# ianwhale/tblup

Hardware: AMD Instinct MI355X
Metric: GBLUP fitness evals/sec (whole node), 2k×50k SNP, DE pop=256; 1/2/4/8 GPUs (higher is better)
Workload: dtype fp4 e2m1 system tiles (exact integer genotype products, fp32 accumulate) + f64 Cholesky/solve; 1 GPU; config2: 2000 animals x 50000 SNPs, panel k=1000, DE pop 256 (256 per GPU), n_train=1280, n_valid=320, h2=0.4; pop_total=256, pop_per_gpu=256, parallelism=population sharded over 1 GPU(s) (strong scaling)

## Files before the change

tblup_amd/csrc/capi.hip:

```cpp
#include <algorithm>
#include <cmath>
#include <cstdio>
#include <cstdlib>
#include <cstring>
#include <map>
#include <memory>
#include <string>
#include <unordered_map>
#include <vector>

#include "capi_ctx.h"
#include "mt_jump.h"

using namespace tblup;

namespace tblup_capi {

thread_local std::string g_err;

int fail(int code, const std::string& msg) {
  g_err = msg;
  return code;
}

// ... 423 lines not shown
  const double tri = (double)d.nT * (d.nT + 1) / 2.0 + (double)d.nV * d.nT;
  for (int64_t b = 0; b < B; ++b) {
    const int64_t k = h_off[b + 1] - h_off[b];
    grm_flops += 2.0 * (double)k * tri;
    gather_bytes += 0.5 * (double)k * (double)(d.nT + d.nV);
    stats_bytes += 16.0 * (double)k;
  }
  const int64_t pk_row = (sd.form == FORM_DUAL) ? dual_pk_row(sd) : 0;
  const int64_t pstride = sd.prow * pk_row;
  uint8_t* panel = cv.take<uint8_t>((size_t)B * pstride);
  double* u = cv.take<double>((size_t)B * sd.prow);
  double* scal = cv.take<double>((size_t)B * SCAL);
  double* L = cv.take<double>((size_t)B * l_stride(sd.NT));
  double* Dinv = cv.take<double>((size_t)B * sd.NT * NPACK * BLKD);
  double* z = cv.take<double>((size_t)B * d.nt * sd.ns);
  double* wv = cv.take<double>((size_t)B * d.nt * sd.ns);
  double* rhs = cv.take<double>((size_t)B * d.nt * sd.ns);
  double* Sp = cv.take<double>((size_t)B * TBLUP_NSLOT * 36 * 256);
  const bool use_st = sys_tiles(c, d, sd) && rq.mode != ChunkMode::DebugK && !ft.gsh;
  double* Kdg = cv.take<double>((size_t)B * sd.NT * NPACK * BLKD);
  int16_t* kdb = use_st ? cv.take<int16_t>((size_t)B * sd.NT * KD_TILE) : nullptr;
  int16_t* kcb = use_st ? cv.take<int16_t>((size_t)B * sd.NT * (sd.NT - 1) / 2 * KC_TILE) : nullptr;
  double* Pp = uses_part(c, B, sd.NT, sys_tiles(c, d, sd)) ? cv.take<double>((size_t)2 * B * sd.NT * TILE * TILE) : nullptr;
  double* Qb = use_last_term(c, sd, B) ? cv.take<double>((size_t)B * NPACK * BLKD) : nullptr;
  const bool fold_share = use_st && sd.form == FORM_PRIMAL && ft.nf > 1 && ft.share;
  if (int rc = ws_check(c, cv)) return rc;
  cl.d = d; cl.sd = sd; cl.B = B; cl.off = rq.d_off; cl.idx = rq.d_idx;
  cl.L = L; cl.Dinv = Dinv; cl.z = z; cl.w = wv; cl.rhs = rhs; cl.S = Sp; cl.u = u; cl.scal = scal;
  cl.Kd = Kdg; cl.kd = kdb; cl.kc = kcb; cl.part = Pp; cl.q = Qb;
  cl.yT = (const double*)rq.sp->yT.p; cl.panel = panel; cl.pstride = pstride; cl.gs_row = d.nRp; cl.gpk_row = d.nRp / 4;
  cl.skip = dbg_skip(c) | (rq.mode == ChunkMode::DebugL ? FLAG_WRITE_LJJ : 0);
  cl.padskip = (sd.form == FORM_PRIMAL && sd.pad_first) ? 1 : 0;
  cl.sys_st = c->sys_st;
  std::vector<OffPlan> plan(sd.NT);
  for (int J = 0; J < sd.NT; ++J) {
    plan[J] = plan_of(c, B, sd.NT, J, use_st);
    if (ft.gsh) plan[J].ne = 0;
  }
  const int32_t* csA = (const int32_t*)c->colsum_all.p;
  const bool fuse_stats = !redo && use_st && sd.form == FORM_PRIMAL && (fold_share || sys_tiles_grid(cl) > 0);
  const StatsFuse sf{csA, d.n, d.nT, rq.branch, rq.h2, rq.d_h2, (int32_t*)c->status.p + ST_INDEX, scal, u, rhs};
  int rc = 0;
  if (!redo && !fuse_stats)
    rc = timed(c, s, KC_STATS, 2.0 * (double)h_off[B], stats_bytes, [&] {
      return launch_indiv_stats(d_idx, d_off, B, ft, csA, d, sd, rq.branch, rq.h2, rq.d_h2, scal, u, rhs,
                                (int32_t*)c->status.p + ST_INDEX, s);
    });
  if (rc) return rc;
  if (sd.form == FORM_DUAL && !redo) {
    rc = timed(c, s, KC_GATHER, 0.0, gather_bytes, [&] {
      return launch_gather(ft, d_idx, d_off, pstride, B, csA, scal, d, pk_row, panel, u, s);
    });
    if (rc) return rc;
  }
  res.z = z;
  if (rq.mode == ChunkMode::DebugK) {
    double* K = cv.take<double>((size_t)B * d.nRp * d.nTp);
    if (int rc2 = ws_check(c, cv)) return rc2;
    res.K = K;
    const double kbytes = (double)B * ((double)d.nT * d.nT / 2.0 + (double)d.nV * d.nT) * 8.0;
    return timed(c, s, KC_GRM, grm_flops, kbytes + gather_bytes / 2.0,
                 [&] { return launch_grm(panel, pstride, pk_row, d_off, u, scal, d, B, K, s); });
  }
  res.K = L;
  const double T3 = (double)TILE * TILE * TILE;
  uint64_t* wgt = nullptr;
// ... 180 lines not shown
  if (hipGetDeviceCount(&ndev) != hipSuccess || ndev == 0) return fail(TBLUP_ERR_HIP, "no HIP device available");
  if (device < 0 || device >= ndev) return fail(TBLUP_ERR_ARG, "device id out of range");
  HIPCHK(hipSetDevice(device));
  std::unique_ptr<tblup_ctx> c(new tblup_ctx());
  c->device = device;
  c->n = n;
  c->P = P;
  if (panel) c->pheno.assign(pheno, pheno + n);
  c->nt = 1;
  HIPCHK(hipStreamCreateWithFlags(&c->stream, hipStreamNonBlocking));
  const char* env = getenv("TBLUP_WORKSPACE_MB");
  c->budget = (size_t)(env ? atoll(env) : 32768) << 20;
#ifdef TBLUP_DIAG_BUILD
  const char* dbg = getenv("TBLUP_DBG_SKIP");
  c->dbg_skip = dbg ? atoi(dbg) : 0;
#endif
  const char* wt = getenv("TBLUP_WG_TRACE");
  c->wg_trace = wt && atoi(wt) != 0;
  const char* fp = getenv("TBLUP_FORM");
  c->form_pref = fp ? std::max(0, std::min(2, atoi(fp))) : 0;
  if (const char* e = getenv("TBLUP_AHEAD")) c->ahead = std::max(-1, std::min(1, atoi(e)));
  if (const char* e = getenv("TBLUP_SOLVE_CHAIN")) c->solve_chain = std::max(-1, std::min(1, atoi(e)));
  if (const char* e = getenv("TBLUP_SOLVE_PULL")) c->solve_pull = std::max(-1, std::min(1, atoi(e)));
  if (const char* e = getenv("TBLUP_CHAIN_SYNC")) c->chain_sync = atoi(e);
  if (const char* e = getenv("TBLUP_LAST_TERM")) c->last_term = std::max(-1, std::min(1, atoi(e)));
  if (const char* e = getenv("TBLUP_LT_MASK")) c->lt_mask = (int)strtol(e, nullptr, 0);
  if (const char* e = getenv("TBLUP_FOLD_FUSE")) c->fold_fuse = atoi(e) != 0;
  if (const char* e = getenv("TBLUP_FOLD_SHARE")) c->fold_share = atoi(e) != 0;
  if (const char* e = getenv("TBLUP_SYS_ST")) c->sys_st = std::max(-1, std::min(1, atoi(e)));
  if (const char* e = getenv("TBLUP_FOLD_GSHARE")) c->fold_gshare = atoi(e) != 0;
  if (const char* e = getenv("TBLUP_DUAL_ST")) c->dual_st = atoi(e) != 0;
  if (const char* e = getenv("TBLUP_DIAG_D")) c->diag_d = std::max(-1, std::min(1, atoi(e)));
  if (const char* e = getenv("TBLUP_DIAG_E")) c->diag_e = std::max(-1, std::min(2, atoi(e)));
  if (const char* e = getenv("TBLUP_PAD_FIRST")) c->pad_first = atoi(e) != 0;
  if (const char* e = getenv("TBLUP_RELIAB_LDS")) c->reliab_lds = atoi(e) != 0;
  if (const char* e = getenv("TBLUP_SCORE_LDS")) c->score_lds = atoi(e) != 0;
  if (const char* e = getenv("TBLUP_NRS")) c->nrs = (atoi(e) == 1 || atoi(e) == 2 || atoi(e) == 4) ? atoi(e) : 0;
  if (const char* e = getenv("TBLUP_CHAIN_DEBUG")) {
    int sp = 0, dl = 0, sh = 0;
    if (sscanf(e, "%d,%d,%d", &sp, &dl, &sh) == 3 && sp > 0 && dl >= 0 && sh > 0) {
      c->chain_dbg_spin = sp;
      c->chain_dbg_delay = dl;
      c->chain_dbg_shots = sh;
    }
  }
  if (!panel) {
    *out = c.release();
    return 0;
  }
  const size_t gbytes = (size_t)n * (size_t)P;
  if (int rc = dev_alloc(c.get(), c->geno_sm, gbytes)) return rc;
  if (int rc = dev_alloc(c.get(), c->colsum_all, (size_t)P * 4)) return rc;
  if (int rc = dev_alloc(c.get(), c->status, ST_WORDS * 4)) return rc;
  HIPCHK(hipMemsetAsync(c->status.p, 0, ST_WORDS * 4, c->stream));
  if (layout == TBLUP_LAYOUT_SNP_MAJOR) {
    HIPCHK(hipMemcpyAsync(c->geno_sm.p, geno, gbytes, hipMemcpyHostToDevice, c->stream));
  } else {
    if (int rc = dev_alloc(c.get(), c->scratch, gbytes)) return rc;
    HIPCHK(hipMemcpyAsync(c->scratch.p, geno, gbytes, hipMemcpyHostToDevice, c->stream));
    HIPCHK(launch_transpose_geno((const int8_t*)c->scratch.p, (int8_t*)c->geno_sm.p, n, P, c->stream));
  }
  HIPCHK(launch_colsum_all((const int8_t*)c->geno_sm.p, (int32_t*)c->colsum_all.p, n, P, c->stream));
  HIPCHK(hipStreamSynchronize(c->stream));
  dev_free(c.get(), c->scratch);
  *out = c.release();
  return 0;
// ... 639 lines not shown
```

tblup_amd/csrc/capi_ctx.h:

```cpp
#pragma once
#include <functional>
#include <map>
#include <memory>
#include <string>
#include <vector>

#include "../../include/tblup_gpu.h"
#include "tblup_internal.h"

struct tblup_ctx;

namespace tblup_capi {

int fail(int code, const std::string& msg);

#define HIPCHK(expr)                                                                                      \
  do {                                                                                                    \
    hipError_t e_ = (expr);                                                                               \
    if (e_ != hipSuccess) return fail(TBLUP_ERR_HIP, std::string(#expr) + ": " + hipGetErrorString(e_)); \
  } while (0)

inline int64_t round_up(int64_t x, int64_t m) { return (x + m - 1) / m * m; }

struct DevBuf {
// ... 41 lines not shown
  DevBuf dec_keys, dec_idx;
  DevBuf de_polys, de_small, de_par, de_chi;
  int64_t de_L = -1, de_pop = -1;
  bool de_end_jump = false;
  uint32_t* de_host = nullptr;
  char* de_stage = nullptr;
  size_t de_stage_bytes = 0;
  hipEvent_t de_ev = nullptr;
  bool de_pending = false;
  DevBuf mde_dev;
  std::vector<uint32_t> mde_key;
  int32_t mde_pos = -1;
  int64_t mde_cmax = 0;
  int64_t mde_pop = -1, mde_L = -1, mde_scr = 0;
  size_t budget = 0;
  bool profiling = false;
  std::vector<EventPair> pending;
  std::vector<hipEvent_t> event_pool;
  double ms[TBLUP_N_KCLASS] = {0};
  int64_t launches[TBLUP_N_KCLASS] = {0};
  double flops[TBLUP_N_KCLASS] = {0};
  double bytes[TBLUP_N_KCLASS] = {0};
  int64_t mem_in_use = 0;

  bool wg_trace = false;
  DevBuf wgt;
  int64_t wgt_used = 0;
  int dbg_skip = 0;
  int form_pref = 0;
  int ahead = -1;
  int nrs = 0;
  int diag_d = -1;
  int diag_e = -1;
  int chain_sync = 0;
  int last_term = -1;
  int lt_mask = -1;
  int solve_chain = -1;
  int solve_pull = -1;
  int fold_fuse = 1;
  int fold_share = 1;
  int fold_gshare = 1;
  int dual_st = 1;
  std::vector<int32_t> gmap_host;
  int sys_st = -1;
  int pad_first = 1;
  int reliab_lds = 1;
  int score_lds = 1;
  std::vector<int64_t> fold_hoff;
  DevBuf chain;
  int32_t chain_seq = 0;
  bool host_entry = false;
  int64_t chain_recoveries = 0;
  int32_t chain_dbg_spin = 0, chain_dbg_delay = 0, chain_dbg_shots = 0;
};

namespace tblup_capi {
int dev_alloc(tblup_ctx* c, DevBuf& b, size_t bytes);
void dev_free(tblup_ctx* c, DevBuf& b);
int check_ctx(tblup_ctx* c);
void clear_error();

struct Carve {
  char* base;
  size_t used = 0;
  template <typename T>
  T* take(size_t count) {
// ... 48 lines not shown
```

tblup_amd/csrc/k_chol.hip:

```cpp
#include "chol_dev.h"
#include <algorithm>
#include <type_traits>

namespace tblup {

namespace {

constexpr int BKD = 16;
constexpr int LTS = BKD * TILE;
constexpr int TT = TILE * TILE;

__device__ __forceinline__ v4d mfma64(double a, double b, v4d c) {
  return __builtin_amdgcn_mfma_f64_16x16x4f64(a, b, c, 0, 0, 0);
}
__device__ __forceinline__ v4d mfma64_nega(double a, double b, v4d c) {
  return __builtin_amdgcn_mfma_f64_16x16x4f64(a, b, c, 0, 0, 1);
}

constexpr int NSLOT = TBLUP_NSLOT;

typedef __attribute__((address_space(3))) void* lds_ptr_t;


__device__ __forceinline__ int lt_off(int k, int x) { return k * TILE + 2 * ((x >> 1) ^ (8 * (k & 1))) + (x & 1); }
// ... 138 lines not shown
                                         double* dst) {
  const int l = threadIdx.x & 63;
  const double* sc = a.scal + b * SCAL;
  const double sa = sc[SC_SA], cN = sc[SC_CN], invd = sc[SC_INVD], lam = sc[SC_LAM], sm = sc[SC_SM];
  const int64_t nrow = (int64_t)sc[SC_NROW], pad = (int64_t)sc[SC_PAD];
  int q, sb;
  tri_decode(e, q, sb);
  const int64_t j0 = (int64_t)J * TILE;
  const double* ub = a.u + b * a.prow + j0;
  const int il = 16 * sb + (l & 15);
  const int64_t gj = j0 + il;
  const double uj = ub[il];
  const v4i c4 = unpack_counts4(cv);
#pragma unroll
  for (int r = 0; r < 4; ++r) {
    const int cl = 16 * q + (l >> 4) + 4 * r;
    const int64_t gi = j0 + cl;
    const double kv = grm_value(c4[r], ub[cl], uj, sa, cN, invd, sm);
    const double v = (sys_real(gi, pad, nrow) && sys_real(gj, pad, nrow)) ? kv + ((gi == gj) ? lam : 0.0)
                                                                         : ((gi == gj) ? 1.0 : 0.0);
    double* d = dst + pk(q, sb) + bo((l >> 4) + 4 * r, l & 15);
    __builtin_nontemporal_store(v - sub[r], d);
  }
}
__device__ __forceinline__ int2 kd_load(const CholArgs& a, int64_t b, int J, int e) {
  const int l = threadIdx.x & 63;
  return nt_load2(a.kd + kd_tile(a.NT, b, J) + (e * 64 + l) * 4);
}

__device__ __forceinline__ int skip_rows(const CholArgs& a, int64_t b) {
  return a.padskip ? ((int)a.scal[b * SCAL + SC_PAD] & ~3) : 0;
}

__device__ __forceinline__ void factor16_any(const CholArgs& a, double* D, double* X, int l, uint64_t* st = nullptr) {
  if (a.skip & FLAG_WRITE_LJJ)
    factor16<true>(D, X, l, st);
  else
    factor16<false>(D, X, l, st);
}

__device__ __forceinline__ void dstamp(const CholArgs& a, int slot) {
  if (a.dtr && blockIdx.x == 0 && (threadIdx.x & 63) == 0)
    a.dtr[(threadIdx.x >> 6) * 64 + slot] = __builtin_amdgcn_s_memrealtime();
}

__device__ __forceinline__ int32_t gsh_count(const CholArgs& a, int64_t s, int64_t r, int64_t c) {
  const FoldTab& ft = a.ft;
  const int32_t* mp = ft.gmap + (int64_t)fold_of(ft, s) * ft.gmap_ld;
  const int32_t mr = mp[r], mc = mp[c];
  return (mr >= 0 && mc >= 0) ? ft.gsh[((s % ft.bpf) * ft.gsh_ld + mr) * ft.gsh_ld + mc] : 0;
}

constexpr int DW = 8;
constexpr int DTHR = 64 * DW;
static_assert(DTHR == 4 * TILE, "diag z: four lanes per row");

constexpr int OW = 8;
constexpr int OTH = 64 * OW;

template <int D, int WCL = -1>
__device__ __forceinline__ void i8_tt8_pk64(const uint8_t* sa, const uint8_t* sb, int64_t nblk, uint8_t* lds,
                                            v4i (&cnt)[8]) {
  const int l = threadIdx.x & 63, w = threadIdx.x >> 6;
  const int wc = (WCL < 0) ? w : WCL;
#pragma unroll
  for (int cb = 0; cb < 8; ++cb) cnt[cb] = v4i{0, 0, 0, 0};
  if (nblk <= 0) return;
  const int64_t nst = (nblk + 3) >> 2;
  constexpr int TB = TILE * 64;
  auto issue = [&](int64_t st) {
    uint8_t* slot = lds + (int)(st % D) * 2 * TB;
    glds16_asm(sa + st * 64, slot + w * 1024);
    glds16_asm(sb + st * 64, slot + TB + w * 1024);
  };
  for (int64_t st = 0; st < D - 1 && st < nst; ++st) issue(st);
  const int rho = l & 15, prow = (rho >> 2) + 4 * (rho & 3), ch = l >> 4;
  const int tail_ch = (int)(nblk & 3);
  for (int64_t st = 0; st < nst; ++st) {
    if (st + D - 2 < nst) {
      asm volatile("s_waitcnt vmcnt(%0)" ::"n"((D - 2) * 2) : "memory");
    } else {
      asm volatile("s_waitcnt vmcnt(0)" ::: "memory");
    }
    __builtin_amdgcn_s_barrier();
    if (st + D - 1 < nst) issue(st + D - 1);
    const uint8_t* As = lds + (int)(st % D) * 2 * TB;
    const uint8_t* Bs = As + TB;
    uint4 bq = *reinterpret_cast<const uint4*>(Bs + i8off_b(16 * wc + rho, ch));
// ... 316 lines not shown
  for (; lb + 1 < q; lb += 2) {
    const double* A0 = Tp + pk(q, lb);
    const double* B0 = Xp + pk(lb, jb);
    const double* A1 = Tp + pk(q, lb + 1);
    const double* B1 = Xp + pk(lb + 1, jb);
#pragma unroll
    for (int kk = 0; kk < 4; ++kk) {
      const int k = 4 * kk + (l >> 4);
      s0 = mfma64(A0[bo(l & 15, k)], B0[bo(k, l & 15)], s0);
      s1 = mfma64(A1[bo(l & 15, k)], B1[bo(k, l & 15)], s1);
    }
  }
  if (lb < q) {
    const double* A0 = Tp + pk(q, lb);
    const double* B0 = Xp + pk(lb, jb);
#pragma unroll
    for (int kk = 0; kk < 4; ++kk) {
      const int k = 4 * kk + (l >> 4);
      s0 = mfma64(A0[bo(l & 15, k)], B0[bo(k, l & 15)], s0);
    }
  }
  const v4d sacc = s0 + s1;
  v4d xo = {0.0, 0.0, 0.0, 0.0};
  const double* Xqq = Xp + pk(q, q);
#pragma unroll
  for (int kk = 0; kk < 4; ++kk) xo = mfma64_nega(Xqq[bo(l & 15, 4 * kk + (l >> 4))], sacc[kk], xo);
  double* dst = Xp + pk(q, jb);
#pragma unroll
  for (int r = 0; r < 4; ++r) dst[bo((l >> 4) + 4 * r, l & 15)] = xo[r];
}

template <int NTR>
__device__ __forceinline__ void diag_z(const CholArgs& a, const double* Xp, const double (*rsh)[TILE], int64_t b,
                                       int64_t j0) {
  const int t = threadIdx.x, i = t >> 2, q = t & 3;
  const int qi = i >> 4, ii = i & 15;
  double acc[NTR];
#pragma unroll
  for (int tr = 0; tr < NTR; ++tr) acc[tr] = 0.0;
  for (int c = q; c <= i; c += 4) {
    const double xc = Xp[pk(qi, c >> 4) + bo(ii, c & 15)];
#pragma unroll
    for (int tr = 0; tr < NTR; ++tr) acc[tr] += xc * rsh[tr][c];
  }
#pragma unroll
  for (int tr = 0; tr < NTR; ++tr) {
    double v = acc[tr];
    v += __shfl_xor(v, 1);
    v += __shfl_xor(v, 2);
    if (q == 0) a.z[(b * NTR + tr) * a.ns + j0 + i] = v;
  }
}

__device__ __forceinline__ void diag_tile(const CholArgs& a, int64_t b, int J, int L0, double* lds,
                                          double (*rsh)[TILE]) {
  const int t = threadIdx.x, l = t & 63, w = t >> 6;
  const int64_t ns = a.ns;
  const int NT = a.NT;
  const int64_t j0 = (int64_t)J * TILE;
  const double* sc = a.scal + b * SCAL;
  const double muf = sc[SC_MUF];
  const int64_t nrow = (int64_t)sc[SC_NROW], pad = (int64_t)sc[SC_PAD];
  const int nt = a.nt;
  double* Tp = lds;
  double* Xp = lds + NPACK * BLKD;
  dstamp(a, 0);

  double rv[MAXT] = {0.0, 0.0, 0.0, 0.0};
  const int64_t gi = j0 + t;
  if (t < TILE) {
#pragma unroll
    for (int tr = 0; tr < MAXT; ++tr) {
      if (tr < nt) {
        const int64_t o = (b * nt + tr) * ns + gi;
        const double wv = (J > 0) ? a.w[o] : 0.0;
        const int fo = fold_of(a.ft, b);
        rv[tr] = ((a.form == FORM_PRIMAL) ? a.rhs[o] : a.ft.yT[fo][tr * a.ytp + gi] - muf * a.ft.ymu[fo][tr]) - wv;
      }
    }
  }

  const double* src = (L0 == 0) ? a.Kd + (b * NT + J) * (int64_t)NPACK * BLKD
                                : a.S + (b * NSLOT + (J & 1)) * (int64_t)NPACK * BLKD;
  {
#pragma unroll
    for (int e = 0; e < NPACK * BLKD / 2 / DTHR; ++e) {
      const int chunk = (e * DW + w) * 64;
      __builtin_amdgcn_global_load_lds(src + 2 * (chunk + l), (lds_ptr_t)(Tp + 2 * chunk), 16, 0, 2);
    }
    if (J > L0 && a.q != nullptr) {
      const double* qg = a.q + b * (int64_t)NPACK * BLKD;
#pragma unroll
      for (int e = 0; e < NPACK * BLKD / 2 / DTHR; ++e) {
        const int chunk = (e * DW + w) * 64;
        __builtin_amdgcn_global_load_lds(qg + 2 * (chunk + l), (lds_ptr_t)(Xp + 2 * chunk), 16, 0, 0);
      }
      asm volatile("s_waitcnt vmcnt(0)" ::: "memory");
      __syncthreads();
      for (int e = t; e < NPACK * BLKD; e += DTHR) Tp[e] -= Xp[e];
      __syncthreads();
    } else if (J > L0 && !(a.skip & 2)) {
      v4d acc[5];
#pragma unroll
      for (int i = 0; i < 5; ++i) acc[i] = v4d{0.0, 0.0, 0.0, 0.0};
      syrk_lower8_32(a.L + b * l_stride(NT) + ((int64_t)J * NT + L0) * TT, 8 * (J - L0), Xp, acc);
#pragma unroll
      for (int i = 0; i < 5; ++i) {
        const int e = syrk_e(w, i);
        if (i < syrk_nb(w)) {
          const int q = tri_q_rt(e);
          double* blk = Tp + pk(q, e - q * (q + 1) / 2);
#pragma unroll
          for (int r = 0; r < 4; ++r) blk[bo((l >> 4) + 4 * r, l & 15)] -= acc[i][r];
        }
      }
    }
    asm volatile("s_waitcnt vmcnt(0)" ::: "memory");
  }
#pragma unroll
  for (int e = t; e < NBLK * BLKD; e += DTHR) {
    const int p = e >> 8, o = e & 255, r = o >> 4;
    const int c = 2 * (((o & 15) >> 1) ^ ((r >> 1) & 7)) + (o & 1);
    Xp[pk(p, p) + o] = (c == NB - 1 - r) ? 1.0 : 0.0;
  }
  if (t < TILE) {
#pragma unroll
    for (int tr = 0; tr < MAXT; ++tr) rsh[tr][t] = (tr < nt && sys_real(gi, pad, nrow)) ? rv[tr] : 0.0;
  }
  dstamp(a, 1);
  __syncthreads();
  dstamp(a, 2);

  if (!(a.skip & 4)) {
    if (w == 0 && !(a.skip & 256)) factor16_any(a, Tp + pk(0, 0), Xp + pk(0, 0), l);
    __syncthreads();
  }
  for (int p = 0; p < ((a.skip & 4) ? 0 : NBLK); ++p) {
    for (int q = p + 1 + w; q < ((a.skip & 512) ? 0 : NBLK); q += DW) {
      v4d x = {0.0, 0.0, 0.0, 0.0};
      x = mma_abt(Tp + pk(q, p), Xp + pk(p, p), x, l);
#pragma unroll
      for (int r = 0; r < 4; ++r) Tp[pk(q, p) + bo((l >> 4) + 4 * r, l & 15)] = x[r];
    }
    dstamp(a, 3 + 3 * p);
    __syncthreads();
    if (p + 1 == NBLK) break;
    const int nb = NBLK - 1 - p;
    if (w == 0) {
      uint64_t* st = (a.dtr && blockIdx.x == 0 && p == 3) ? a.dtr : nullptr;
      fstamp(st, 54);
      if (!(a.skip & 512)) {
        v4d x = {0.0, 0.0, 0.0, 0.0};
        x = mma_abt(Tp + pk(p + 1, p), Tp + pk(p + 1, p), x, l);
        double* dst = Tp + pk(p + 1, p + 1);
#pragma unroll
        for (int r = 0; r < 4; ++r) dst[bo((l >> 4) + 4 * r, l & 15)] -= x[r];
      }
      if (!(a.skip & 256)) factor16_any(a, Tp + pk(p + 1, p + 1), Xp + pk(p + 1, p + 1), l, st);
    } else {
      const int wi = w - 1;
      constexpr int NTW = DW - 1;
      const int ne = (a.skip & 512) ? 0 : nb * (nb + 1) / 2;
      for (int e = wi + 1; e < ne; e += 2 * NTW) {
        const int e2 = e + NTW;
        int qq = 0;
        while ((qq + 1) * (qq + 2) / 2 <= e) ++qq;
        const int q = p + 1 + qq, sb = p + 1 + (e - qq * (qq + 1) / 2);
        const bool two = e2 < ne;
        int qq2 = qq;
        while ((qq2 + 1) * (qq2 + 2) / 2 <= e2) ++qq2;
        const int q2 = two ? p + 1 + qq2 : q, sb2 = two ? p + 1 + (e2 - qq2 * (qq2 + 1) / 2) : sb;
        const double* A = Tp + pk(q, p);
        const double* B = Tp + pk(sb, p);
        const double* A2 = Tp + pk(q2, p);
        const double* B2 = Tp + pk(sb2, p);
        v4d x = {0.0, 0.0, 0.0, 0.0}, x2 = {0.0, 0.0, 0.0, 0.0};
#pragma unroll
        for (int kk = 0; kk < 4; ++kk) {
          const int k = 4 * kk + (l >> 4);
          x = mfma64(A[bo(l & 15, k)], B[bo(l & 15, k)], x);
          x2 = mfma64(A2[bo(l & 15, k)], B2[bo(l & 15, k)], x2);
        }
        double* dst = Tp + pk(q, sb);
#pragma unroll
        for (int r = 0; r < 4; ++r) dst[bo((l >> 4) + 4 * r, l & 15)] -= x[r];
        if (two) {
          double* dst2 = Tp + pk(q2, sb2);
#pragma unroll
          for (int r = 0; r < 4; ++r) dst2[bo((l >> 4) + 4 * r, l & 15)] -= x2[r];
        }
      }
      if (!(a.skip & 8) && wi < p) xinv_block(Tp, Xp, p, wi, l);
    }
    dstamp(a, 4 + 3 * p);
    __syncthreads();
    dstamp(a, 5 + 3 * p);
  }
  if (a.skip & 16) return;

  if (!(a.skip & 4) && !(a.skip & 8)) {
    if (w < NBLK - 1) xinv_block(Tp, Xp, NBLK - 1, w, l);
    dstamp(a, 26);
    __syncthreads();
    dstamp(a, 27);
  }

  {
    double* Xg = a.Dinv + (b * NT + J) * (int64_t)NPACK * BLKD;
    for (int k = t; k < ((a.skip & (1 << 14)) ? 0 : NPACK * BLKD / 2); k += DTHR) {
      const int g = 2 * k, blk = g >> 8, o = g & 255, r = o >> 4;
      const int c0 = 2 * (((o & 15) >> 1) ^ ((r >> 1) & 7));
      const double* xb = Xp + blk * BLKD;
      *reinterpret_cast<v2d*>(Xg + g) = v2d{xb[bo(c0, r)], xb[bo(c0 + 1, r)]};
    }
  }
  if (a.skip & FLAG_WRITE_LJJ) {
    double* Ld = a.L + b * l_stride(NT) + ((int64_t)J * NT + J) * TT;
    for (int e = t; e < TT; e += DTHR) {
      const int rr = e >> 7, cc = e & 127;
      Ld[e] = (cc >= rr) ? Tp[pk(cc >> 4, rr >> 4) + bo(cc & 15, rr & 15)] : 0.0;
    }
  }
  dstamp(a, 28);
  if (!(a.skip & (1 << 15))) {
    switch (nt) {
      case 1: diag_z<1>(a, Xp, rsh, b, j0); break;
      case 2: diag_z<2>(a, Xp, rsh, b, j0); break;
      case 3: diag_z<3>(a, Xp, rsh, b, j0); break;
      default: diag_z<4>(a, Xp, rsh, b, j0); break;
    }
  }
  dstamp(a, 29);
}


template <int NCB>
__device__ __forceinline__ void kc_issue(const CholArgs& a, int64_t b, int I, int Jt, int cb0, int2 (&kcv)[NCB]) {
  const int l = threadIdx.x & 63, w = threadIdx.x >> 6;
  const int16_t* kt = a.kc + kc_tile(a.NT, b, I, Jt) + w * 8 * 64 * 4;
#pragma unroll
  for (int cb = 0; cb < NCB; ++cb) kcv[cb] = nt_load2(kt + ((cb0 + cb) * 64 + l) * 4);
}

__device__ __forceinline__ void k_stage(const CholArgs& a, int64_t b, int64_t i0, int64_t j0, double* pq_sh,
                                        double* ui_sh) {
  const int t = threadIdx.x;
  if (t < TILE) {
    const double* sc = a.scal + b * SCAL;
    const double sa = sc[SC_SA], cN = sc[SC_CN], invd = sc[SC_INVD], sm = sc[SC_SM];
    const int64_t nrow = (int64_t)sc[SC_NROW], pad = (int64_t)sc[SC_PAD];
    const double uj = a.u[b * a.prow + j0 + t];
    const bool rj = sys_real(j0 + t, pad, nrow);
    reinterpret_cast<v2d*>(pq_sh)[t] = rj ? v2d{-invd * (sa + sm * uj), invd * (cN - sa * uj)} : v2d{0.0, 0.0};
    ui_sh[t] = a.u[b * a.prow + i0 + t];
  }
}

template <int NCB, bool GSH = true>
__device__ __forceinline__ void k_acc(const CholArgs& a, int64_t b, int I, int Jt, int cb0, const int2 (&kcv)[NCB],
                                      uint8_t* lds8, const double* pq_sh, const double* ui_sh, v4d (&acc)[NCB]) {
  const int l = threadIdx.x & 63, w = threadIdx.x >> 6;
  const int64_t i0 = (int64_t)I * TILE, j0 = (int64_t)Jt * TILE;
  const double* sc = a.scal + b * SCAL;
  const double invd = sc[SC_INVD];
  const int64_t nrow = (int64_t)sc[SC_NROW], pad = (int64_t)sc[SC_PAD];
// ... 197 lines not shown
  }
  const double* Lb = a.L + b * l_stride(NT);
  if (!(a.skip & 64))
    gemm1_a32<8>(Lb + (int64_t)J * NT * TT + (int64_t)ls0 * TT, Lb + (int64_t)I * NT * TT + (int64_t)ls0 * TT, 1, 0, lds,
                 acc, ls0 == 0 ? skip_rows(a, b) : 0);
#pragma unroll
  for (int cb = 0; cb < 8; ++cb) {
    v2d* d = reinterpret_cast<v2d*>(pd + (cb * 64 + l) * 4);
    __builtin_nontemporal_store(v2d{acc[cb][0], acc[cb][1]}, d);
    __builtin_nontemporal_store(v2d{acc[cb][2], acc[cb][3]}, d + 1);
  }
}

__global__ __launch_bounds__(DTHR) void k_chol_diag(CholArgs a, int64_t ne, int ls0) {
  __shared__ __attribute__((aligned(16))) double lds[2 * NPACK * BLKD];
  __shared__ double rsh[MAXT][TILE];
  WgTrace tr(a.wgt);
  if ((int64_t)blockIdx.x >= a.B) {
    const int64_t x = blockIdx.x - a.B, nd = gridDim.x - a.B - ne;
    if (x < nd) {
      const int64_t b = xcd_remap(x, nd);
      syrk_partial8(a, b, a.J + 1, a.J, lds, 0);
      tr.done(WGT_DPREP, a.J, a.J + 1, b);
    } else {
      const int64_t lg = xcd_remap(x - nd, ne);
      const int64_t b = lg % a.B;
      const int I = a.J + 1 + (int)(lg / a.B);
      e_unit(a, b, I, ls0, lds);
      tr.done(WGT_EPART, a.J, I, b);
    }
    return;
  }
  const int64_t b = xcd_remap(blockIdx.x, a.B);
  diag_tile(a, b, a.J, a.J >= 2 ? a.J - 1 : 0, lds, rsh);
  tr.done(WGT_DIAG, a.J, a.J, b);
}

__device__ __forceinline__ void diag_grm_tile(const CholArgs& a, int64_t b, int J, uint8_t* lds, double* u_sh) {
  const int t = threadIdx.x, l = t & 63, w = t >> 6;
  const int NT = a.NT;
  const int64_t j0 = (int64_t)J * TILE;
  const double* sc = a.scal + b * SCAL;
  const double sa = sc[SC_SA], cN = sc[SC_CN], invd = sc[SC_INVD], lam = sc[SC_LAM], sm = sc[SC_SM];
  const int64_t nrow = (int64_t)sc[SC_NROW], nblk = (int64_t)sc[SC_CBLK], pad = (int64_t)sc[SC_PAD];
  if (t < TILE) u_sh[t] = a.u[b * a.prow + j0 + t];
  double* Kd = a.Kd + (b * NT + J) * (int64_t)NPACK * BLKD;
  v4i cnt[8];
  const int row = 16 * w + (l >> 2), pos = l & 3;
  const int wc = (w < 4) ? w : 11 - w;
#pragma unroll
  for (int cb = 0; cb < 8; ++cb) cnt[cb] = v4i{0, 0, 0, 0};
  if (a.skip & 1) {
    __syncthreads();
  } else if (a.ft.gsh) {
#pragma unroll
    for (int cb = 0; cb < 8; ++cb)
      if (cb >= wc)
#pragma unroll
        for (int r = 0; r < 4; ++r) cnt[cb][r] = gsh_count(a, b, j0 + 16 * cb + (l >> 4) + 4 * r, j0 + 16 * wc + (l & 15));
  } else {
    const uint8_t* rp = a.form == FORM_PRIMAL ? row_packed(a, b, j0 + row) : row_dpk(a, b, j0 + row);
    const uint8_t* sa = rp + pk_swz_a(row, pos);
    const uint8_t* sb = rp + pk_swz_b(row, pos);
    switch (wc) {
      case 0: i8_tt8_pk64<4, 0>(sa, sb, nblk, lds, cnt); break;
      case 1: i8_tt8_pk64<4, 1>(sa, sb, nblk, lds, cnt); break;
      case 2: i8_tt8_pk64<4, 2>(sa, sb, nblk, lds, cnt); break;
// ... 127 lines not shown
  const int row = 16 * w + (l >> 2), pos = l & 3;
  const int64_t nblk = (int64_t)a.scal[b * SCAL + SC_CBLK];
  v4i cnt[8];
  i8_tt8_pk64<4>(row_dpk(a, b, j0 + row) + pk_swz_a(row, pos), row_dpk(a, b, i0 + row) + pk_swz_b(row, pos), nblk, lds,
                 cnt);
  const int64_t ld = a.ft.gsh_ld;
  int32_t* G = a.ft.gsh + b * ld * ld;
  const int64_t ic = i0 + 16 * w + (l & 15);
#pragma unroll
  for (int cb = 0; cb < 8; ++cb)
#pragma unroll
    for (int r = 0; r < 4; ++r) {
      const int64_t jr = j0 + 16 * cb + (l >> 4) + 4 * r;
      G[jr * ld + ic] = cnt[cb][r];
      G[ic * ld + jr] = cnt[cb][r];
    }
}

hipError_t launch_gshare(const CholLaunch& c, hipStream_t s) {
  const FoldTab& ft = c.ft;
  if (!ft.gsh || c.sd.form != FORM_DUAL || c.d.nRp % TILE) return hipErrorInvalidValue;
  CholArgs a = make_args(c, 0);
  a.wgt = nullptr;
  const int NR = (int)(c.d.nRp / TILE);
  hipLaunchKernelGGL(k_gshare, dim3((unsigned)(ft.bpf * NR * (NR + 1) / 2)), dim3(OTH), 0, s, a, NR);
  return hipGetLastError();
}

hipError_t launch_chol_diag(const CholLaunch& c, int J, const OffPlan& p, hipStream_t s) {
  CholArgs a = make_args(c, J);
  const int64_t nwg = c.B * (1 + p.ndd) + p.ne;
  if (p.ne > 0 && (c.part == nullptr || J < 1 || p.ne > c.B * p.nI || c.ft.gsh)) return hipErrorInvalidValue;
  if (c.wgt) a.dtr = c.wgt + nwg * WGT_REC;
  hipLaunchKernelGGL(k_chol_diag, dim3((unsigned)nwg), dim3(DTHR), 0, s, a, p.ne, p.ahead_cur ? J - 1 : 0);
  return hipGetLastError();
}

hipError_t launch_chol_offdiag(const CholLaunch& c, int J, const OffPlan& p, hipStream_t s) {
  if (p.nI <= 0) return hipSuccess;
  CholArgs a = make_args(c, J);
  if (c.d.nt == 1)
    hipLaunchKernelGGL(k_chol_offdiag<1>, dim3((unsigned)offdiag_grid(p, c.B)), dim3(OTH), 0, s, a, p);
  else
    hipLaunchKernelGGL(k_chol_offdiag<MAXT>, dim3((unsigned)offdiag_grid(p, c.B)), dim3(OTH), 0, s, a, p);
  return hipGetLastError();
}

}
```

tblup_amd/csrc/tblup_internal.h:

```cpp
#pragma once
#include <hip/hip_runtime.h>
#include <cstdint>

namespace tblup {

constexpr int TILE = 128;
constexpr int TBLUP_NSLOT = 2;
constexpr int KBLK = 64;
constexpr int MAXT = 4;
constexpr int GATHER_ROWS = 128;

constexpr int SCAL = 16;
enum {
  SC_SA = 0,
  SC_CN = 1,
  SC_INVD = 2,
  SC_MUF = 3,
  SC_LAM = 4,
  SC_D = 5,
  SC_MODE = 6,
  SC_K = 7,
  SC_SM = 8,
  SC_NROW = 9,
  SC_CBLK = 10,
// ... 104 lines not shown
  double* rhs;
};
constexpr int64_t L_PAD = 512;
__host__ __device__ inline int64_t l_stride(int NT) { return (int64_t)NT * NT * TILE * TILE + L_PAD; }
struct CholLaunch {
  EvalDims d;
  SysDims sd;
  int64_t B;
  double* L;
  double* Dinv;
  double* z;
  double* w;
  const double* rhs;
  double* S;
  double* Kd;
  const double* yT;
  const uint8_t* panel;
  int64_t pstride;
  const int64_t* off;
  const int64_t* idx;
  int64_t gs_row;
  int64_t gpk_row;
  FoldTab ft;
  const double* u;
  const double* scal;
  int skip;
  uint64_t* wgt;
  int16_t* kc;
  double* part;
  double* q;
  int padskip;
  int16_t* kd;
  int sys_st = -1;
  const StatsFuse* stats = nullptr;
};
constexpr int64_t KC_TILE = (int64_t)TILE * TILE;
constexpr int64_t KD_TILE = (int64_t)NPACK * BLKD;
constexpr int64_t KC_MAX_NT = 8191;
constexpr int WGT_REC = 4;
constexpr int DTR_RECS = 8 * 64 / WGT_REC;
enum { WGT_DIAG = 1, WGT_TILE = 2, WGT_PREP = 3, WGT_KJJ = 4, WGT_SYS = 5, WGT_PART = 6, WGT_DPREP = 9, WGT_EPART = 10 };
struct OffPlan {
  int nI, nP, nrs, nds, ahead_cur;
  int ndd;
  int64_t n_kd;
  int64_t ne;
  __host__ __device__ int64_t units() const { return (int64_t)nP * nrs + nds + nI; }
};
constexpr int64_t AHEAD_SLOTS = 256;
constexpr int64_t DD_MIN_B = 64;
constexpr int64_t DD_MAX_B = 128;
constexpr int DD_MAX_J = 3;
OffPlan off_plan(int64_t B, int NT, int J, bool sys_tiles, int ahead, int nrs, int64_t slots = AHEAD_SLOTS,
                 int diag_d = 0, int dd_maxj = DD_MAX_J, int diag_e = 0, int64_t ncu = 0);
int cu_count();
inline int64_t offdiag_grid(const OffPlan& p, int64_t B) { return p.nI > 0 ? B * p.units() + p.n_kd : 0; }
hipError_t launch_chol_diag(const CholLaunch& c, int J, const OffPlan& p, hipStream_t s);
hipError_t launch_chol_offdiag(const CholLaunch& c, int J, const OffPlan& p, hipStream_t s);
hipError_t launch_diag_grm(const CholLaunch& c, hipStream_t s);
hipError_t launch_gshare(const CholLaunch& c, hipStream_t s);
hipError_t launch_sys_tiles(const CholLaunch& c, hipStream_t s);
int64_t sys_tiles_grid(const CholLaunch& c);
constexpr int SP_ROWTAB = 4096;
hipError_t launch_sys_tiles_folds(const CholLaunch& c, hipStream_t s);
struct SolveChain {
  int32_t* flags;
  double* beta;
  double* cpart;
  double* epart;
  double* mbpart;
  int32_t* err;
  int32_t* expired;
  int32_t seq;
  int32_t mode;
  int32_t spin_max;
  int32_t pull;
  int32_t delay;
};
constexpr int32_t CHAIN_SPIN_MAX = 1 << 20;
constexpr int CHAIN_ERR_RING = 64;
enum { ST_INDEX = 0, ST_SOLVE = 1, ST_WORDS = 2 };
__host__ __device__ inline int64_t chain_flags(int NT) { return (int64_t)NT * (NT + 2); }
hipError_t launch_solve(const CholLaunch& c, const SolveChain* ch, double* fitness, double* ebv, hipStream_t s);
hipError_t launch_effects(const CholLaunch& c, const int32_t* csA, double* center, double* effects, int64_t plane,
                          hipStream_t s);

constexpr int RELIAB_W = 16;
// ... 73 lines not shown
```

Before: 110,500 evals/s.

## Add wide 16-wave diagonal Cholesky kernel overlapping inverse store and z computation

Adds a templated diag_tile with a 16-wave workgroup variant, launched by default when the plan has no extra diagonal or part work. Extra waves take over the Dinv row stores and per-row diag_z products and interleave them with the blocked factorization loop, instead of running them as a serial tail after factorization. Non-working waves join syrk barriers as bystanders. This aims to shorten the latency-bound diagonal tile step, at the cost of more complex wave-role bookkeeping, more LDS and register pressure per workgroup, and lower occupancy.

After: 112,100 evals/s (median of 6 runs). 1.01x the previous value.

```diff
diff --git a/tblup_amd/csrc/capi.hip b/tblup_amd/csrc/capi.hip
--- a/tblup_amd/csrc/capi.hip
+++ b/tblup_amd/csrc/capi.hip
@@ -479,6 +479,7 @@
   cl.skip = dbg_skip(c) | (rq.mode == ChunkMode::DebugL ? FLAG_WRITE_LJJ : 0);
   cl.padskip = (sd.form == FORM_PRIMAL && sd.pad_first) ? 1 : 0;
   cl.sys_st = c->sys_st;
+  cl.diag_waves = c->diag_waves;
   std::vector<OffPlan> plan(sd.NT);
   for (int J = 0; J < sd.NT; ++J) {
     plan[J] = plan_of(c, B, sd.NT, J, use_st);
@@ -725,6 +726,7 @@
   if (const char* e = getenv("TBLUP_DUAL_ST")) c->dual_st = atoi(e) != 0;
   if (const char* e = getenv("TBLUP_DIAG_D")) c->diag_d = std::max(-1, std::min(1, atoi(e)));
   if (const char* e = getenv("TBLUP_DIAG_E")) c->diag_e = std::max(-1, std::min(2, atoi(e)));
+  if (const char* e = getenv("TBLUP_DIAG_WAVES")) c->diag_waves = (atoi(e) == 8 || atoi(e) == 12 || atoi(e) == 16) ? atoi(e) : 0;
   if (const char* e = getenv("TBLUP_PAD_FIRST")) c->pad_first = atoi(e) != 0;
   if (const char* e = getenv("TBLUP_RELIAB_LDS")) c->reliab_lds = atoi(e) != 0;
   if (const char* e = getenv("TBLUP_SCORE_LDS")) c->score_lds = atoi(e) != 0;
diff --git a/tblup_amd/csrc/capi_ctx.h b/tblup_amd/csrc/capi_ctx.h
--- a/tblup_amd/csrc/capi_ctx.h
+++ b/tblup_amd/csrc/capi_ctx.h
@@ -97,6 +97,7 @@
   int nrs = 0;
   int diag_d = -1;
   int diag_e = -1;
+  int diag_waves = 0;
   int chain_sync = 0;
   int last_term = -1;
   int lt_mask = -1;
diff --git a/tblup_amd/csrc/k_chol.hip b/tblup_amd/csrc/k_chol.hip
--- a/tblup_amd/csrc/k_chol.hip
+++ b/tblup_amd/csrc/k_chol.hip
@@ -194,8 +194,9 @@
   return a.padskip ? ((int)a.scal[b * SCAL + SC_PAD] & ~3) : 0;
 }
 
+template <bool LJJ = true>
 __device__ __forceinline__ void factor16_any(const CholArgs& a, double* D, double* X, int l, uint64_t* st = nullptr) {
-  if (a.skip & FLAG_WRITE_LJJ)
+  if (LJJ && (a.skip & FLAG_WRITE_LJJ))
     factor16<true>(D, X, l, st);
   else
     factor16<false>(D, X, l, st);
@@ -215,7 +216,11 @@
 
 constexpr int DW = 8;
 constexpr int DTHR = 64 * DW;
-static_assert(DTHR == 4 * TILE, "diag z: four lanes per row");
+constexpr int DWX = DIAG_WAVES_WIDE;
+static_assert(DWX > DW && DWX % 4 == 0 && DWX <= 16, "wide diagonal workgroup: 12 or 16 waves");
+static_assert(64 == 4 * NB && DW >= NBLK, "diag z: four lanes per row, one wave per block row");
+
+
 
 constexpr int OW = 8;
 constexpr int OTH = 64 * OW;
@@ -598,14 +603,25 @@
 
 template <int NTR>
 __device__ __forceinline__ void diag_z(const CholArgs& a, const double* Xp, const double (*rsh)[TILE], int64_t b,
-                                       int64_t j0) {
-  const int t = threadIdx.x, i = t >> 2, q = t & 3;
-  const int qi = i >> 4, ii = i & 15;
+                                       int64_t j0, int qr) {
+  const int l = threadIdx.x & 63, ii = l >> 2, i = 16 * qr + ii, q = l & 3;
   double acc[NTR];
 #pragma unroll
   for (int tr = 0; tr < NTR; ++tr) acc[tr] = 0.0;
-  for (int c = q; c <= i; c += 4) {
-    const double xc = Xp[pk(qi, c >> 4) + bo(ii, c & 15)];
+#pragma unroll 1
+  for (int cb = 0; cb < qr; ++cb) {
+    const double* xb = Xp + pk(qr, cb);
+    double xc[4];
+#pragma unroll
+    for (int j = 0; j < 4; ++j) xc[j] = xb[bo(ii, q + 4 * j)];
+#pragma unroll
+    for (int j = 0; j < 4; ++j) {
+#pragma unroll
+      for (int tr = 0; tr < NTR; ++tr) acc[tr] += xc[j] * rsh[tr][16 * cb + q + 4 * j];
+    }
+  }
+  for (int c = 16 * qr + q; c <= i; c += 4) {
+    const double xc = Xp[pk(qr, qr) + bo(ii, c & 15)];
 #pragma unroll
     for (int tr = 0; tr < NTR; ++tr) acc[tr] += xc * rsh[tr][c];
   }
@@ -617,10 +633,53 @@
     if (q == 0) a.z[(b * NTR + tr) * a.ns + j0 + i] = v;
   }
 }
-
+__device__ __forceinline__ void diag_z_row(const CholArgs& a, const double* Xp, const double (*rsh)[TILE], int64_t b,
+                                           int64_t j0, int qr) {
+  if (a.skip & (1 << 15)) return;
+  switch (a.nt) {
+    case 1: diag_z<1>(a, Xp, rsh, b, j0, qr); break;
+    case 2: diag_z<2>(a, Xp, rsh, b, j0, qr); break;
+    case 3: diag_z<3>(a, Xp, rsh, b, j0, qr); break;
+    default: diag_z<4>(a, Xp, rsh, b, j0, qr); break;
+  }
+}
+
+__device__ __forceinline__ void dinv_store_row(const CholArgs& a, const double* Xp, double* Xg, int qr, int tid,
+                                               int nthr) {
+  if (a.skip & (1 << 14)) return;
+  const int k0 = pk(qr, 0) / 2, k1 = pk(qr, qr + 1) / 2;
+  for (int k = k0 + tid; k < k1; k += nthr) {
+    const int g = 2 * k, blk = g >> 8, o = g & 255, r = o >> 4;
+    const int c0 = 2 * (((o & 15) >> 1) ^ ((r >> 1) & 7));
+    const double* xb = Xp + blk * BLKD;
+    *reinterpret_cast<v2d*>(Xg + g) = v2d{xb[bo(c0, r)], xb[bo(c0 + 1, r)]};
+  }
+}
+
+__device__ __forceinline__ void syrk_lower8_32_bystander(int nst16, int r0 = 0) {
+  const int nst = nst16 >> 1, s0 = r0 >> 5, kf = (r0 & 31) >> 2;
+  if (nst <= s0) return;
+  int s = s0;
+  if (kf > 0) {
+    __builtin_amdgcn_s_barrier();
+    ++s;
+  }
+  for (; s < nst; ++s) __builtin_amdgcn_s_barrier();
+  __syncthreads();
+}
+
+template <int NW>
+__device__ __forceinline__ int diag_rank(int w) {
+  if constexpr (NW == DW) return w - 1;
+  return (w & 3) ? 3 * (w >> 2) + (w & 3) - 1 : 3 * (NW / 4) + (w >> 2) - 1;
+}
+
+template <int NW>
 __device__ __forceinline__ void diag_tile(const CholArgs& a, int64_t b, int J, int L0, double* lds,
                                           double (*rsh)[TILE]) {
+  constexpr int NTHR = 64 * NW;
   const int t = threadIdx.x, l = t & 63, w = t >> 6;
+  const int wu = __builtin_amdgcn_readfirstlane(w);
   const int64_t ns = a.ns;
   const int NT = a.NT;
   const int64_t j0 = (int64_t)J * TILE;
@@ -648,43 +707,52 @@
 
   const double* src = (L0 == 0) ? a.Kd + (b * NT + J) * (int64_t)NPACK * BLKD
                                 : a.S + (b * NSLOT + (J & 1)) * (int64_t)NPACK * BLKD;
+  const bool aw = NW == DW || wu < DW;
   {
-#pragma unroll
-    for (int e = 0; e < NPACK * BLKD / 2 / DTHR; ++e) {
-      const int chunk = (e * DW + w) * 64;
-      __builtin_amdgcn_global_load_lds(src + 2 * (chunk + l), (lds_ptr_t)(Tp + 2 * chunk), 16, 0, 2);
+    if (aw) {
+#pragma unroll
+      for (int e = 0; e < NPACK * BLKD / 2 / DTHR; ++e) {
+        const int chunk = (e * DW + w) * 64;
+        __builtin_amdgcn_global_load_lds(src + 2 * (chunk + l), (lds_ptr_t)(Tp + 2 * chunk), 16, 0, 2);
+      }
     }
     if (J > L0 && a.q != nullptr) {
       const double* qg = a.q + b * (int64_t)NPACK * BLKD;
-#pragma unroll
-      for (int e = 0; e < NPACK * BLKD / 2 / DTHR; ++e) {
-        const int chunk = (e * DW + w) * 64;
-        __builtin_amdgcn_global_load_lds(qg + 2 * (chunk + l), (lds_ptr_t)(Xp + 2 * chunk), 16, 0, 0);
+      if (aw) {
+#pragma unroll
+        for (int e = 0; e < NPACK * BLKD / 2 / DTHR; ++e) {
+          const int chunk = (e * DW + w) * 64;
+          __builtin_amdgcn_global_load_lds(qg + 2 * (chunk + l), (lds_ptr_t)(Xp + 2 * chunk), 16, 0, 0);
+        }
       }
       asm volatile("s_waitcnt vmcnt(0)" ::: "memory");
       __syncthreads();
-      for (int e = t; e < NPACK * BLKD; e += DTHR) Tp[e] -= Xp[e];
+      for (int e = t; e < NPACK * BLKD; e += NTHR) Tp[e] -= Xp[e];
       __syncthreads();
     } else if (J > L0 && !(a.skip & 2)) {
-      v4d acc[5];
-#pragma unroll
-      for (int i = 0; i < 5; ++i) acc[i] = v4d{0.0, 0.0, 0.0, 0.0};
-      syrk_lower8_32(a.L + b * l_stride(NT) + ((int64_t)J * NT + L0) * TT, 8 * (J - L0), Xp, acc);
-#pragma unroll
-      for (int i = 0; i < 5; ++i) {
-        const int e = syrk_e(w, i);
-        if (i < syrk_nb(w)) {
-          const int q = tri_q_rt(e);
-          double* blk = Tp + pk(q, e - q * (q + 1) / 2);
-#pragma unroll
-          for (int r = 0; r < 4; ++r) blk[bo((l >> 4) + 4 * r, l & 15)] -= acc[i][r];
+      if (aw) {
+        v4d acc[5];
+#pragma unroll
+        for (int i = 0; i < 5; ++i) acc[i] = v4d{0.0, 0.0, 0.0, 0.0};
+        syrk_lower8_32(a.L + b * l_stride(NT) + ((int64_t)J * NT + L0) * TT, 8 * (J - L0), Xp, acc);
+#pragma unroll
+        for (int i = 0; i < 5; ++i) {
+          const int e = syrk_e(w, i);
+          if (i < syrk_nb(w)) {
+            const int q = tri_q_rt(e);
+            double* blk = Tp + pk(q, e - q * (q + 1) / 2);
+#pragma unroll
+            for (int r = 0; r < 4; ++r) blk[bo((l >> 4) + 4 * r, l & 15)] -= acc[i][r];
+          }
         }
+      } else {
+        syrk_lower8_32_bystander(8 * (J - L0));
       }
     }
     asm volatile("s_waitcnt vmcnt(0)" ::: "memory");
   }
 #pragma unroll
-  for (int e = t; e < NBLK * BLKD; e += DTHR) {
+  for (int e = t; e < NBLK * BLKD; e += NTHR) {
     const int p = e >> 8, o = e & 255, r = o >> 4;
     const int c = 2 * (((o & 15) >> 1) ^ ((r >> 1) & 7)) + (o & 1);
     Xp[pk(p, p) + o] = (c == NB - 1 - r) ? 1.0 : 0.0;
@@ -697,38 +765,47 @@
   __syncthreads();
   dstamp(a, 2);
 
+  const int rk = diag_rank<NW>(wu);
+  constexpr int NWK = NW - 1;
+  constexpr int ZR = NW == DW ? NWK - 1 : 3 * (NW / 4) - 1;
+  double* Xg = a.Dinv + (b * NT + J) * (int64_t)NPACK * BLKD;
+  constexpr int LR = NBLK - 1;
+  auto upd_next = [&](int p) {
+    v4d x = {0.0, 0.0, 0.0, 0.0};
+    x = mma_abt(Tp + pk(p + 1, p), Tp + pk(p + 1, p), x, l);
+    double* dst = Tp + pk(p + 1, p + 1);
+#pragma unroll
+    for (int r = 0; r < 4; ++r) dst[bo((l >> 4) + 4 * r, l & 15)] -= x[r];
+  };
   if (!(a.skip & 4)) {
-    if (w == 0 && !(a.skip & 256)) factor16_any(a, Tp + pk(0, 0), Xp + pk(0, 0), l);
+    if (wu == 0 && !(a.skip & 256)) factor16_any<NW == DW>(a, Tp + pk(0, 0), Xp + pk(0, 0), l);
     __syncthreads();
   }
-  for (int p = 0; p < ((a.skip & 4) ? 0 : NBLK); ++p) {
-    for (int q = p + 1 + w; q < ((a.skip & 512) ? 0 : NBLK); q += DW) {
+  for (int p = 0; p + 1 < ((a.skip & 4) ? 0 : NBLK); ++p) {
+    const int qc = (wu == 0) ? p + 1 : p + 2 + rk;
+    if (qc < ((a.skip & 512) ? 0 : NBLK)) {
       v4d x = {0.0, 0.0, 0.0, 0.0};
-      x = mma_abt(Tp + pk(q, p), Xp + pk(p, p), x, l);
-#pragma unroll
-      for (int r = 0; r < 4; ++r) Tp[pk(q, p) + bo((l >> 4) + 4 * r, l & 15)] = x[r];
+      x = mma_abt(Tp + pk(qc, p), Xp + pk(p, p), x, l);
+#pragma unroll
+      for (int r = 0; r < 4; ++r) Tp[pk(qc, p) + bo((l >> 4) + 4 * r, l & 15)] = x[r];
     }
     dstamp(a, 3 + 3 * p);
     __syncthreads();
-    if (p + 1 == NBLK) break;
     const int nb = NBLK - 1 - p;
-    if (w == 0) {
+    if (wu == 0) {
       uint64_t* st = (a.dtr && blockIdx.x == 0 && p == 3) ? a.dtr : nullptr;
       fstamp(st, 54);
-      if (!(a.skip & 512)) {
-        v4d x = {0.0, 0.0, 0.0, 0.0};
-        x = mma_abt(Tp + pk(p + 1, p), Tp + pk(p + 1, p), x, l);
-        double* dst = Tp + pk(p + 1, p + 1);
-#pragma unroll
-        for (int r = 0; r < 4; ++r) dst[bo((l >> 4) + 4 * r, l & 15)] -= x[r];
-      }
-      if (!(a.skip & 256)) factor16_any(a, Tp + pk(p + 1, p + 1), Xp + pk(p + 1, p + 1), l, st);
+      if (!(a.skip & 512)) upd_next(p);
+      if (!(a.skip & 256)) factor16_any<NW == DW>(a, Tp + pk(p + 1, p + 1), Xp + pk(p + 1, p + 1), l, st);
     } else {
-      const int wi = w - 1;
-      constexpr int NTW = DW - 1;
+      int ti = rk, ntw = NWK;
+      if constexpr (NW != DW) {
+        ntw = ZR - p;
+        ti = (rk < ZR) ? rk - p : -1;
+      }
       const int ne = (a.skip & 512) ? 0 : nb * (nb + 1) / 2;
-      for (int e = wi + 1; e < ne; e += 2 * NTW) {
-        const int e2 = e + NTW;
+      for (int e = ti + 1; ti >= 0 && e < ne; e += 2 * ntw) {
+        const int e2 = e + ntw;
         int qq = 0;
         while ((qq + 1) * (qq + 2) / 2 <= e) ++qq;
         const int q = p + 1 + qq, sb = p + 1 + (e - qq * (qq + 1) / 2);
@@ -756,7 +833,12 @@
           for (int r = 0; r < 4; ++r) dst2[bo((l >> 4) + 4 * r, l & 15)] -= x2[r];
         }
       }
-      if (!(a.skip & 8) && wi < p) xinv_block(Tp, Xp, p, wi, l);
+      if (!(a.skip & 8) && rk < p) xinv_block(Tp, Xp, p, rk, l);
+      if (p >= 1 && !(a.skip & 8)) {
+        if (NW == DW && rk == ZR) dinv_store_row(a, Xp, Xg, p - 1, l, 64);
+        if (NW != DW && rk > ZR) dinv_store_row(a, Xp, Xg, p - 1, 64 * (rk - ZR - 1) + l, 64 * (NWK - 1 - ZR));
+        if (rk == ZR) diag_z_row(a, Xp, rsh, b, j0, p - 1);
+      }
     }
     dstamp(a, 4 + 3 * p);
     __syncthreads();
@@ -765,38 +847,30 @@
   if (a.skip & 16) return;
 
   if (!(a.skip & 4) && !(a.skip & 8)) {
-    if (w < NBLK - 1) xinv_block(Tp, Xp, NBLK - 1, w, l);
+    const int jb = (NW == DW) ? wu : (wu == 0 ? LR : rk);
+    if (jb < LR) xinv_block(Tp, Xp, LR, jb, l);
+    if (NW == DW && wu == NW - 1) dinv_store_row(a, Xp, Xg, LR - 1, l, 64);
+    if (NW != DW && (wu == 0 || rk >= LR))
+      dinv_store_row(a, Xp, Xg, LR - 1, 64 * (wu == 0 ? 0 : rk - LR + 1) + l, 64 * (NW - LR));
     dstamp(a, 26);
     __syncthreads();
     dstamp(a, 27);
   }
 
-  {
-    double* Xg = a.Dinv + (b * NT + J) * (int64_t)NPACK * BLKD;
-    for (int k = t; k < ((a.skip & (1 << 14)) ? 0 : NPACK * BLKD / 2); k += DTHR) {
-      const int g = 2 * k, blk = g >> 8, o = g & 255, r = o >> 4;
-      const int c0 = 2 * (((o & 15) >> 1) ^ ((r >> 1) & 7));
-      const double* xb = Xp + blk * BLKD;
-      *reinterpret_cast<v2d*>(Xg + g) = v2d{xb[bo(c0, r)], xb[bo(c0 + 1, r)]};
-    }
-  }
-  if (a.skip & FLAG_WRITE_LJJ) {
+  if (NW == DW && (a.skip & FLAG_WRITE_LJJ)) {
     double* Ld = a.L + b * l_stride(NT) + ((int64_t)J * NT + J) * TT;
-    for (int e = t; e < TT; e += DTHR) {
+    for (int e = t; e < TT; e += NTHR) {
       const int rr = e >> 7, cc = e & 127;
       Ld[e] = (cc >= rr) ? Tp[pk(cc >> 4, rr >> 4) + bo(cc & 15, rr & 15)] : 0.0;
     }
   }
+  if (wu == NW - 1)
+    diag_z_row(a, Xp, rsh, b, j0, LR - 1);
+  else if (wu == NW - 2)
+    diag_z_row(a, Xp, rsh, b, j0, LR);
+  else
+    dinv_store_row(a, Xp, Xg, LR, t, 64 * (NW - 2));
   dstamp(a, 28);
-  if (!(a.skip & (1 << 15))) {
-    switch (nt) {
-      case 1: diag_z<1>(a, Xp, rsh, b, j0); break;
-      case 2: diag_z<2>(a, Xp, rsh, b, j0); break;
-      case 3: diag_z<3>(a, Xp, rsh, b, j0); break;
-      default: diag_z<4>(a, Xp, rsh, b, j0); break;
-    }
-  }
-  dstamp(a, 29);
 }
 
 
@@ -1060,7 +1134,17 @@
     return;
   }
   const int64_t b = xcd_remap(blockIdx.x, a.B);
-  diag_tile(a, b, a.J, a.J >= 2 ? a.J - 1 : 0, lds, rsh);
+  diag_tile<DW>(a, b, a.J, a.J >= 2 ? a.J - 1 : 0, lds, rsh);
+  tr.done(WGT_DIAG, a.J, a.J, b);
+}
+
+template <int NW>
+__global__ __launch_bounds__(64 * NW) void k_chol_diag_w(CholArgs a) {
+  __shared__ __attribute__((aligned(16))) double lds[2 * NPACK * BLKD];
+  __shared__ double rsh[MAXT][TILE];
+  WgTrace tr(a.wgt);
+  const int64_t b = xcd_remap(blockIdx.x, a.B);
+  diag_tile<NW>(a, b, a.J, a.J >= 2 ? a.J - 1 : 0, lds, rsh);
   tr.done(WGT_DIAG, a.J, a.J, b);
 }
 
@@ -1254,7 +1338,10 @@
   const int64_t nwg = c.B * (1 + p.ndd) + p.ne;
   if (p.ne > 0 && (c.part == nullptr || J < 1 || p.ne > c.B * p.nI || c.ft.gsh)) return hipErrorInvalidValue;
   if (c.wgt) a.dtr = c.wgt + nwg * WGT_REC;
-  hipLaunchKernelGGL(k_chol_diag, dim3((unsigned)nwg), dim3(DTHR), 0, s, a, p.ne, p.ahead_cur ? J - 1 : 0);
+  if (diag_waves(p, c.diag_waves) == DWX && !(a.skip & FLAG_WRITE_LJJ))
+    hipLaunchKernelGGL(k_chol_diag_w<DWX>, dim3((unsigned)nwg), dim3(64 * DWX), 0, s, a);
+  else
+    hipLaunchKernelGGL(k_chol_diag, dim3((unsigned)nwg), dim3(DTHR), 0, s, a, p.ne, p.ahead_cur ? J - 1 : 0);
   return hipGetLastError();
 }
 
diff --git a/tblup_amd/csrc/tblup_internal.h b/tblup_amd/csrc/tblup_internal.h
--- a/tblup_amd/csrc/tblup_internal.h
+++ b/tblup_amd/csrc/tblup_internal.h
@@ -160,13 +160,14 @@
   int padskip;
   int16_t* kd;
   int sys_st = -1;
+  int diag_waves = 0;
   const StatsFuse* stats = nullptr;
 };
 constexpr int64_t KC_TILE = (int64_t)TILE * TILE;
 constexpr int64_t KD_TILE = (int64_t)NPACK * BLKD;
 constexpr int64_t KC_MAX_NT = 8191;
 constexpr int WGT_REC = 4;
-constexpr int DTR_RECS = 8 * 64 / WGT_REC;
+constexpr int DTR_RECS = 16 * 64 / WGT_REC;
 enum { WGT_DIAG = 1, WGT_TILE = 2, WGT_PREP = 3, WGT_KJJ = 4, WGT_SYS = 5, WGT_PART = 6, WGT_DPREP = 9, WGT_EPART = 10 };
 struct OffPlan {
   int nI, nP, nrs, nds, ahead_cur;
@@ -181,6 +182,11 @@
 constexpr int DD_MAX_J = 3;
 OffPlan off_plan(int64_t B, int NT, int J, bool sys_tiles, int ahead, int nrs, int64_t slots = AHEAD_SLOTS,
                  int diag_d = 0, int dd_maxj = DD_MAX_J, int diag_e = 0, int64_t ncu = 0);
+constexpr int DIAG_WAVES_WIDE = 16;
+inline int diag_waves(const OffPlan& p, int knob) {
+  if (p.ndd > 0 || p.ne > 0) return 8;
+  return knob == 8 ? 8 : DIAG_WAVES_WIDE;
+}
 int cu_count();
 inline int64_t offdiag_grid(const OffPlan& p, int64_t B) { return p.nI > 0 ? B * p.units() + p.n_kd : 0; }
 hipError_t launch_chol_diag(const CholLaunch& c, int J, const OffPlan& p, hipStream_t s);
```
